# EBonura/bonnie-32

Measured on AMD Instinct MI355X. Metric: Mtriangles/s + Mpixels/s, 1M-tri synthetic scene @ 2560x1920, higher is better.
Workload: dtype f32+i32 (exact-order f32 setup/barycentrics, integer snap and RGB555 colour tail); 1 GPU; C3: 1000000 tris @ 2560x1920, 256x256 8-bit atlas, affine+snap+RGB555 dither, painter's; triangles_drawn=485525, fragments=9622635, parallelism=single GPU

## Files before the change

### bonnie-32_amd/csrc/b32_api.hip

```cpp
#include "b32_host.h"

extern "C" {

const char* b32_strerror(int code) {
    switch (code) {
        case B32_OK: return "ok";
        case B32_E_ARG: return "invalid argument";
        case B32_E_INDEX: return "face references a vertex index out of range";
        case B32_E_NAN_KEY: return "NaN painter's-sort key";
        case B32_E_HIP: return "HIP runtime error";
        case B32_E_UNSUPPORTED: return "setting outside the supported hot-path scope";
        case B32_E_NO_DEVICE: return "no HIP device (the rasterizer has no CPU fallback)";
        case B32_E_FRAME_DROPPED: return "an earlier frame in flight ran out of buffer space and drew nothing (deep asynchronous mode)";
        case B32_E_BAND_TIMEOUT: return "a band exchange wait gave up: another rank did not publish / release its frame in time (the frame may hold stale rows)";
        default: return "unknown error";
    }
}

int b32_create(int device, b32_ctx** out) {
    if (!out) return B32_E_ARG;
    *out = nullptr;
    int n = 0;
    if (hipGetDeviceCount(&n) != hipSuccess || n <= 0 || device < 0 || device >= n) return B32_E_NO_DEVICE;
    b32_ctx* c = new b32_ctx();
// ... 32 lines not shown
    if (c->side) (void)hipStreamDestroy(c->side);
    if (c->ev_created) for (auto& fr : c->ev) for (auto& e : fr) if (e) (void)hipEventDestroy(e);
    c->lines.release(); c->prims.release(); c->world.release(); c->gizmo.release();
    if (c->world_counts) (void)hipFree(c->world_counts);
    if (c->gizmo_counts) (void)hipFree(c->gizmo_counts);
    for (hipEvent_t e : c->world_ev) if (e) (void)hipEventDestroy(e);
    c->pick_tab.release();
    if (c->pick_words) (void)hipFree(c->pick_words);
    if (c->pick_host) (void)hipHostFree(c->pick_host);
    for (hipEvent_t e : c->pick_tev) if (e) (void)hipEventDestroy(e);
    if (c->hover_bits) (void)hipFree(c->hover_bits);
    if (c->hover_words) (void)hipFree(c->hover_words);
    for (hipEvent_t e : c->hover_tev) if (e) (void)hipEventDestroy(e);
    if (c->own_stream) (void)hipStreamDestroy(c->own_stream);
    if (c->stage_host) (void)hipHostFree(c->stage_host);
    for (hipEvent_t e : c->dl_ev) if (e) (void)hipEventDestroy(e);
    if (c->dl_stream) { (void)hipStreamSynchronize(c->dl_stream); (void)hipStreamDestroy(c->dl_stream); }
    for (hipEvent_t e : c->dl_snap) if (e) (void)hipEventDestroy(e);
    for (uint32_t* q : c->dl_stage) if (q) (void)hipFree(q);
    for (uint32_t k = 0; k < b32_ctx::PICK_RING; ++k) {
        if (c->pick_res[k]) (void)hipFree(c->pick_res[k]);
        for (hipEvent_t e : { c->pick_done[k], c->pick_left[k] }) if (e) (void)hipEventDestroy(e);
    }
    delete c;
}

int b32_last_hip_error(const b32_ctx* c) { return c ? c->last_hip : 0; }
#ifndef B32_SRC_DIGEST
#define B32_SRC_DIGEST "unknown-digest!!"
#endif
// ... 651 lines not shown
    if (c->hover_timed && k < cap && hipEventSynchronize(c->hover_tev[1]) == hipSuccess &&
        hipEventElapsedTime(&hover_ms, c->hover_tev[0], c->hover_tev[1]) == hipSuccess) {
        names[k] = "hover"; ms[k] = hover_ms; ++k;
    }
    return (int)k;
}

}

extern "C" int b32_set_fragment_counting(b32_ctx* c, int on) {
    if (!c) return B32_E_ARG;
    c->count_fragments = on ? 1 : 0;
    return B32_OK;
}
extern "C" unsigned long long b32_route_count(const b32_ctx* c, int which) {
    if (c && which == 7) return c->pipelined_frames;
    if (c && which == 8) return c->lds_atlas_frames;
    if (c && which == 9) return c->wire_tile_frames;
    if (c && which == 10) return c->span_cover_frames;
    if (c && which == 11) return c->flag_join_frames;
    if (c && which == 12) return c->event_join_frames;
    if (c && which == 13) return c->poll_join_frames;
    if (c && which == 14) return c->lines.tile_batches;
    if (c && which == 15) return c->lines.scan_batches;
    if (c && which == 16) return c->prims.tile_batches;
    if (c && which == 17) return c->prims.scan_batches;
    if (c && which == 18) return c->world_tile_batches;
    if (c && which == 19) return c->world_scan_batches;
    return (c && which >= 0 && which < 8) ? c->routes[which] : 0ull;
}
// ... 84 lines not shown
```

### bonnie-32_amd/csrc/b32_device.h

```cpp
#pragma once
#include <hip/hip_runtime.h>
#include <stdint.h>
#include "../../include/b32raster.h"

namespace b32 {

constexpr int TILE_W = 64;
constexpr int TILE_H = 64;
constexpr int TILE_STRIDE = 72;
constexpr int FILL_THREADS = 1024;
constexpr int FILL_WAVES = FILL_THREADS / 64;
constexpr uint32_t KEY_INVALID = 0xFFFFFFFFu;

namespace K {
constexpr int      FRAC_BITS = 12;
constexpr float    ONE_F = (float)(1 << FRAC_BITS);
constexpr uint32_t UNR_ENTRIES = 257, UNR_INDEX_OFFSET = 256, UNR_NUMERATOR = 262144, UNR_ROUND_ADD = 1, UNR_ROUND_DIV = 2;
constexpr int32_t  UNR_SUBTRACT = 257;
constexpr uint32_t DIV_D16_SHIFT = 16, DIV_INDEX_SHIFT = 7, DIV_INDEX_MAX = 256, DIV_NR1_SHIFT = 8, DIV_NR2_SHIFT = 8, DIV_SHIFT_BASE = 36;
constexpr uint64_t DIV_INDEX_BIAS = 0x7FC0, DIV_U_ADD = 0x101, DIV_NR1_CONST = 0x2000080, DIV_NR2_CONST = 0x80;
constexpr float    PF_DISTANCE = 5.0f, PF_SCALE = 4.0f, PF_VIEWPORT_DIV = 2.0f, PF_VIEWPORT_FRAC = 0.75f;
constexpr int32_t  PF_DENOM_GUARD = 256;
constexpr float    P_DISTANCE = 5.0f, P_US_SUB = 1.0f, P_VIEWPORT_DIV = 2.0f, P_VIEWPORT_FRAC = 0.75f, P_DENOM_GUARD = 0.001f;
constexpr float    NEAR_PLANE = 0.1f;
// ... 102 lines not shown
    uint32_t pairs_overflow;
    uint32_t tile_cursor;
    uint32_t list_demand;
    uint32_t need_global_sort;
    uint32_t wire_overflow;
    uint32_t sticky;
    unsigned long long fragments;
};

struct Stamps { unsigned long long t[8]; };
struct Events { uint32_t bad_index, nan_opaque, nan_transparent, overflow, long_transparent, setup_done ,
                join_abort ,
                fill_started ,
                wbin_done ,
                poll_done ,
                poll_lost , _pad[5]; };
__device__ __forceinline__ Events* events_of(Ctrl* ctrl) { return reinterpret_cast<Events*>(reinterpret_cast<unsigned char*>(ctrl) + 128); }
enum { ST_SETUP = 0, ST_BIN = 1, ST_FILL = 2, ST_WIRE = 3, ST_END = 4,
       ST_CLK0 = 5, ST_CLK1 = 6, ST_CLKW = 7 };
__device__ __forceinline__ void phase_stamp(Ctrl* ctrl, int k) {
    if (blockIdx.x == 0 && threadIdx.x == 0) {
        unsigned long long* t = reinterpret_cast<Stamps*>(ctrl + 1)->t;
        if (!t[k]) t[k] = wall_clock64();
    }
}

constexpr uint32_t LOCAL_SORT_CAP = 2048;

struct CamFx {
    int32_t px, py, pz, bx[3], by[3], bz[3];
    int32_t vs, half_w, half_h;
// ... 292 lines not shown
    const uint32_t* spans;
    const uint32_t* partials;
    const uint32_t* texmask;
    uint32_t mask_lds_words;
    uint32_t clear_on, clear_rgba;
    uint32_t clear_depth;
    uint32_t narrow_only;
    const uint8_t* atlas0;
    uint32_t atlas_idx_bytes;
    uint32_t stagger;
    uint32_t span_cover;
    uint32_t join_seq, join_patience;
    uint32_t start_seq;
    uint32_t start_defer;
    uint32_t prio64;
#ifdef B32_TIMELINE
    unsigned long long* dbg;
#endif
};
void launch_fill(hipStream_t s, const FillArgs& a, int n_cu, hipEvent_t after_cover = nullptr);
size_t fill_lds_tex_budget();
constexpr uint32_t ATLAS_CLUT_BYTES = 512;
uint32_t fill_lds_atlas_room(bool wide);

}
```

### bonnie-32_amd/csrc/b32_fill.hip

```cpp
#include "b32_cover.h"
#include "b32_shade_tile.h"

namespace b32 {

constexpr uint32_t RQ_WORDS = 64, RQ_BYTES = RQ_WORDS * 4;
static_assert(2 * (4 * LDS_TILE_BYTES + LDS_MISC_BYTES + 8 * RQ_BYTES + 511) / 512 * 512 <= 160 * 1024, "two 8-wave workgroups per CU");

template <int NT>
__device__ __forceinline__ void reduce_setup_counters(const FillArgs& a, uint32_t* misc, uint32_t tid, uint32_t lane) {
    if (tid < 5) misc[8 + tid] = 0;
    __syncthreads();
    const uint32_t npart = (a.fp.nf + 255) / 256;
    uint32_t acc[5] = { 0, 0, 0, 0, 0 };
    for (uint32_t b = tid; b < npart; b += NT)
#pragma unroll
        for (int k = 0; k < 5; ++k) acc[k] += a.partials[b * 8 + k];
#pragma unroll
    for (int k = 0; k < 5; ++k) {
        const uint32_t tot = (uint32_t)__builtin_amdgcn_readlane((int)dpp_add_scan(acc[k]), 63);
        if (lane == 0 && tot) atomicAdd(&misc[8 + k], tot);
    }
    __syncthreads();
    if (tid == 0) {
        const uint32_t t[5] = { misc[8], misc[9], misc[10], misc[11], misc[12] };
// ... 35 lines not shown
    if (tid == 0) {
        Events* ev = events_of(a.ctrl);
        const unsigned long long t0 = wall_clock64();
        uint32_t lost = 0, waited = 0;
        while (__hip_atomic_fetch_add(&ev->poll_done, 0u, __ATOMIC_RELAXED, __HIP_MEMORY_SCOPE_AGENT) != a.join_seq) {
            if (wall_clock64() - t0 > (unsigned long long)a.join_patience) { lost = 1; break; }
            waited = 1;
            __builtin_amdgcn_s_sleep(32);
        }
        if (lost) { atomicOr(&a.ctrl->sticky, 8u); (void)__hip_atomic_exchange(&ev->poll_lost, a.join_seq, __ATOMIC_RELAXED, __HIP_MEMORY_SCOPE_AGENT); }
        if (waited) __builtin_amdgcn_fence(__ATOMIC_ACQUIRE, "agent");
        misc[7] = lost;
    }
    __syncthreads();
    return misc[7] != 0;
}

template <int NT>
__device__ __forceinline__ TexDesc stage_texture(const FillArgs& a, unsigned char* dst_bytes, uint32_t tid) {
    const TexDesc lds_desc = a.tex[0];
    const uint4* src = reinterpret_cast<const uint4*>(a.texels + lds_desc.offset);
    uint4* dst = reinterpret_cast<uint4*>(dst_bytes);
    const uint32_t nq = (a.lds_tex_texels + 7) / 8;
    for (uint32_t i = tid; i < nq; i += NT) dst[i] = src[i];
    return lds_desc;
}

template <int NT>
__device__ __forceinline__ void leave_undrawn(const FillArgs& a, uint32_t ntiles, uint32_t tid, uint32_t redraw, bool publish) {
    if (a.direct_bin) {
// ... 187 lines not shown
    const bool join_lost = (P64 && a.join_seq) ? join_setup(a, misc, tid) : false;
    phase_stamp(a.ctrl, ST_FILL);
    uint32_t pre_span = 0xFFFFFFFFu, pre_key = 0u;
    if (P64 && a.inline_bin && tid < fp.nf && !join_lost) { pre_span = a.spans[tid]; if (a.gather_blend) pre_key = a.keys[tid]; }
    if (P64 && EXACT && a.mask_lds_words) {
        uint32_t* ml = tilebuf + 2 * TILE_H * TILE_STRIDE;
        for (uint32_t i = tid; i < a.mask_lds_words; i += NT) ml[i] = a.texmask[i];
        ltex = reinterpret_cast<const uint16_t*>(ml);
    }
    bool reduce_late = false;
    if (P64 && (a.inline_bin || a.direct_bin)) {
        bool reduce = a.inline_bin != 0, join_abort = join_lost;
        uint32_t redraw = 0;
        if (a.direct_bin) {
            const Events* ev = events_of(a.ctrl);
            reduce = ev->bad_index == a.epoch || ev->nan_opaque == a.epoch || ev->nan_transparent == a.epoch;
            redraw = (ev->overflow == a.epoch ? 2u : 0u) | (ev->long_transparent == a.epoch ? 1u : 0u);
            join_abort = join_lost || ev->join_abort == a.epoch;
            reduce_late = !reduce && blockIdx.x == 0;
        }
        if (tid == 0) misc[6] = 0;
        __syncthreads();
        if (reduce && !join_abort) reduce_setup_counters<NT>(a, misc, tid, lane);
        if (join_abort) {
            leave_undrawn<NT>(a, ntiles, tid, 0u, false);
            return;
        }
        if (misc[6] || redraw) {
            leave_undrawn<NT>(a, ntiles, tid, redraw, !misc[6]);
            return;
        }
    } else {
        if (a.ctrl->abort || (P64 && a.ctrl->need_global_sort)) {
// ... 66 lines not shown
    }
#ifdef B32_TIMELINE
    if (P64 && a.dbg && lane < 32 && B32_DBG_SLOTS(tilebuf)[lane]) atomicAdd(a.dbg + 1 + 4 * 8192 + lane, B32_DBG_SLOTS(tilebuf)[lane]);
#endif
    if (P64 && blockIdx.x == 0 && tid == 0) {
        unsigned long long* st = reinterpret_cast<Stamps*>(a.ctrl + 1)->t;
        st[ST_CLK0] = clk_entry; st[ST_CLK1] = (unsigned long long)clock64(); st[ST_CLKW] = wall_clock64();
    }
    if (P64 && reduce_late) { __syncthreads(); reduce_setup_counters<NT>(a, misc, tid, lane); }
    if (EXACT && !ZMODE) publish_fragments<NW>(a, smem, frag_count, tid, lane, wave);
}

template <int TEXMODE, bool EXACT, int NT, bool ZMODE, bool FMT8 = false, bool P64 = false, int PLAIN = 0>
__global__ __launch_bounds__(NT) __attribute__((amdgpu_waves_per_eu((P64 && NT == 512 && !PLAIN) ? B32_P64_WAVES : 4))) void k_cover(FillArgs a_in) {
    cover_body<TEXMODE, EXACT, NT, ZMODE, FMT8, P64, PLAIN>(a_in);
}

#ifndef B32_PLAIN_CAP
#define B32_PLAIN_CAP 56
#endif
__global__ __launch_bounds__(512) __attribute__((amdgpu_waves_per_eu(4), amdgpu_num_vgpr(B32_PLAIN_CAP))) void k_cover_plain(FillArgs a_in) {
    cover_body<0, false, 512, false, false, true, 1>(a_in);
}
__global__ __launch_bounds__(512) __attribute__((amdgpu_waves_per_eu(4), amdgpu_num_vgpr(56))) void k_cover_plain_z(FillArgs a_in) {
    cover_body<0, false, 512, true, false, true, 1>(a_in);
}
__global__ __launch_bounds__(512) __attribute__((amdgpu_waves_per_eu(4), amdgpu_num_vgpr(56))) void k_cover_plain8(FillArgs a_in) {
    cover_body<0, false, 512, false, true, true, 2>(a_in);
}
#ifndef B32_LIT_VGPR
#define B32_LIT_VGPR 56
#endif
__global__ __launch_bounds__(512) __attribute__((amdgpu_waves_per_eu(4), amdgpu_num_vgpr(B32_LIT_VGPR))) void k_cover_lit(FillArgs a_in) {
    cover_body<0, false, 512, true, false, true, 3>(a_in);
}

#ifdef B32_TIMELINE
static unsigned long long* g_timeline = nullptr;
extern "C" int b32_debug_timeline(unsigned long long* out, unsigned cap_words) {
    if (!g_timeline) return 0;
    (void)hipDeviceSynchronize();
    (void)hipMemcpy(out, g_timeline, (size_t)cap_words * 8, hipMemcpyDeviceToHost);
    return 1;
}
#endif
template <bool EXACT, bool ZMODE, bool FMT8>
static void launch_p64(hipStream_t s, const FillArgs& a_in, uint32_t ntiles, int n_cu, bool wide) {
    FillArgs a = a_in;
    const size_t atlas = a.atlas_idx_bytes ? (((size_t)ATLAS_CLUT_BYTES + a.atlas_idx_bytes + 15) & ~(size_t)15) : 0;
// ... 115 lines not shown
```

### bonnie-32_amd/csrc/b32_frame.hip

```cpp
#include "b32_host.h"

static void swap_with(b32_ctx* c, FrameSet& a) { std::swap(c->cur, a); }
static void rotate_sets(b32_ctx* c) {
    swap_with(c, c->alt[0]);
    if (c->n_sets == 3) std::swap(c->alt[0], c->alt[1]);
}
static void unrotate_sets(b32_ctx* c) {
    if (c->n_sets == 3) std::swap(c->alt[0], c->alt[1]);
    swap_with(c, c->alt[0]);
}
static int pipeline_ensure(b32_ctx* c) {
    if (!c->side) {
        int prio_least = 0, prio_greatest = 0;
        (void)hipDeviceGetStreamPriorityRange(&prio_least, &prio_greatest);
        HIPCHK(c, hipStreamCreateWithPriority(&c->side, hipStreamNonBlocking, prio_least));
        HIPCHK(c, hipEventCreateWithFlags(&c->ev_main, hipEventDisableTiming));
        HIPCHK(c, hipEventCreateWithFlags(&c->ev_wbin, hipEventDisableTiming));
        HIPCHK(c, hipEventCreateWithFlags(&c->cur.ev_setup, hipEventDisableTiming));
        for (FrameSet& a : c->alt) HIPCHK(c, hipEventCreateWithFlags(&a.ev_setup, hipEventDisableTiming));
        c->side_dirty = true;
    }
    for (uint32_t k = 0; k + 1 < c->n_sets; ++k) {
        FrameSet& a = c->alt[k];
        if (!a.d_ctrl) {
            HIPCHK(c, hipMalloc(reinterpret_cast<void**>(&a.d_ctrl), sizeof(Ctrl) + sizeof(Stamps) + sizeof(Events)));
            HIPCHK(c, hipMemsetAsync(a.d_ctrl, 0, sizeof(Ctrl) + sizeof(Stamps) + sizeof(Events), c->stream));
            c->side_dirty = true;
        }
        if (a.cap_work < c->cap_work || !a.crecs) {
            HIPCHK(c, hipStreamSynchronize(c->stream));
            a.release();
            const size_t n = c->cap_work;
            int rc;
            if ((rc = ensure_plain(c, a.keys0, n))) return rc;
// ... 334 lines not shown
    const bool join_small = !c->frame_batched && (c->join_stream != s || c->join_ok);
    c->pipe_hint = r.direct_bin && (ntiles > 2u * (uint32_t)c->n_cu || c->frame_batched || join_small);
    if (!c->pipe_hint) c->pipelined = false;
    c->last_local_sort = r.local_sort || r.want_prio64;
    c->last_exact = r.ordered_all ? true : (r.exact_cov && !fp.zmode);
    c->last_direct = r.direct_bin;
    if (c->scene.nf == 0) {
        HIPCHK(c, hipMemsetAsync(c->cur.d_ctrl, 0, offsetof(Ctrl, sticky), s));
        HIPCHK(c, hipMemsetAsync(&c->cur.d_ctrl->fragments, 0, sizeof(unsigned long long), s));
        HIPCHK(c, hipMemsetAsync(c->cur.d_ctrl + 1, 0, sizeof(Stamps), s));
    }
    const float *pos12 = nullptr, *attr12 = nullptr;
    if ((rc = frame_positions(c, fp, pos12, attr12))) return fail(rc);

    hipStream_t ss = s;
    if (c->pipelined) {
        if (c->side_dirty) { HIPCHK(c, hipEventRecord(c->ev_main, s)); HIPCHK(c, hipStreamWaitEvent(c->side, c->ev_main, 0)); c->side_dirty = false; }
        ss = c->side;
        c->pipelined_frames++;
        uint32_t polled_tiles = 0, polled_groups = 0, polled_seq = 0;
        for (const auto& co : c->cover_of) if (co.ctrl && co.ctrl == c->alt[0].d_ctrl) { polled_tiles = co.tiles; polled_groups = co.groups; polled_seq = co.seq; }
        const bool start_gate = polled_tiles && polled_seq && c->alt[0].d_ctrl;
        if (!start_gate) { HIPCHK(c, hipEventRecord(c->ev_main, s)); HIPCHK(c, hipStreamWaitEvent(c->side, c->ev_main, 0)); }
        uint32_t gate_need = 0;
        if (c->gate_permille && polled_tiles && c->alt[0].d_ctrl) {
            const uint32_t groups = polled_groups, tiles = polled_tiles;
            const uint32_t pre = tiles > groups ? tiles - groups : 0u;
            const uint32_t need = c->gate_permille > 1000u ? (uint32_t)((uint64_t)(c->gate_permille - 1000u) * pre / 1000u)
                                                           : pre + (uint32_t)((uint64_t)(c->gate_permille - 1u) * groups / 1000u);
            gate_need = need;
        }
        const uint32_t start_patience = c->start_lost ? 200000u : 200000000u;
        c->start_lost = false;
        if (gate_need || start_gate) launch_gate(ss, c->alt[0].d_ctrl, gate_need, 30000u , start_gate ? polled_seq : 0u, c->cur.d_ctrl, start_patience);
    }
    const bool wire_on = fp.wire_collect && c->scene.nf;
    bool wire_binned = false, wire_polled = false;
    WireArgs wa{};
    if (wire_on) {
        wa.tris = c->cur.wire; wa.nf = c->scene.nf; wa.table_owner = c->wire_owner; wa.table_first = c->wire_first;
        wa.table_mask = c->cap_wire_table ? (uint32_t)(c->cap_wire_table - 1) : 0;
        wa.fb = c->fb; wa.zbuf = (c->zbuf && c->zbuf_valid) ? c->zbuf : nullptr;
        wa.width = c->width; wa.height = c->height; wa.band_y0 = c->band_y0; wa.band_y1 = c->band_y1; wa.ctrl = c->cur.d_ctrl;
        if (++c->wire_seq == 0) c->wire_seq = 1;
        wa.epoch = c->wire_seq;
        if (!(c->route_off & B32_ROUTE_WIRE_TILES) && c->cur.wire_fill && c->band_y1 > c->band_y0) {
            wa.tile_yb = (c->band_y0 / WIRE_TH) * WIRE_TH; wa.tiles_x = (c->width + TILE_W - 1) / TILE_W;
            wa.tiles_y = (c->band_y1 - wa.tile_yb + WIRE_TH - 1) / WIRE_TH;
// ... 4 lines not shown
    launch_setup(ss, fp, c->scene.d_verts, c->scene.d_faces, c->scene.d_tex, c->d_lights, lset, c->frame_table, c->frame_places, RecArrays{ c->cur.crecs, c->cur.srecs, c->cur.xrecs }, r.db, c->cur.shades, c->cur.keys0,
                 r.direct_bin ? nullptr : c->cur.spans , c->cur.partials, c->cur.d_ctrl, c->cur.wire, c->n_cu, pos12, attr12, c->cur.face_of);
    uint32_t poll_seq = 0, poll_patience = 0;
    const bool poll_batched = c->pipelined && c->frame_batched && c->join_ok && (r.direct_bin || r.want_inline) && !wire_front && !r.ordered_all &&
                              ntiles && 8u * ntiles <= 5u * (uint32_t)c->n_cu && !(c->route_off & B32_ROUTE_WIDE_GROUPS);
    if (poll_batched) {
        const bool lose_flag = (c->inject & 1u) != 0;
        c->inject &= ~1u;
        if (++c->join_seq == 0) c->join_seq = 1;
        launch_flag_poll(c->side, c->cur.d_ctrl, lose_flag ? c->join_seq ^ 0x40000000u : c->join_seq);
        poll_seq = c->join_seq; poll_patience = lose_flag ? 200000u : 200000000u;
        c->flag_join_frames++; c->poll_join_frames++;
    } else if (c->pipelined && r.direct_bin && c->join_ok && !c->frame_batched) {
        const bool lose_flag = (c->inject & 1u) != 0;
        c->inject &= ~1u;
        launch_flag(c->side, c->cur.d_ctrl, lose_flag ? c->epoch ^ 0x40000000u : c->epoch);
        launch_join(s, c->cur.d_ctrl, c->epoch, lose_flag ? 200000u : 200000000u );
        c->flag_join_frames++;
    } else if (c->pipelined) {
        hipError_t e1 = hipEventRecord(c->cur.ev_setup, c->side);
        if (e1 == hipSuccess) e1 = hipStreamWaitEvent(s, c->cur.ev_setup, 0);
        if (e1 != hipSuccess) { (void)hipStreamSynchronize(c->side); c->last_hip = (int)e1; return B32_E_HIP; }
        c->event_join_frames++;
    }
    if (c->pipelined && wire_on && wa.tile_fill) {
        launch_wire_bin(c->side, wa, wire_back, wire_front, true);
        if (wire_back) { launch_flag_wbin(c->side, c->cur.d_ctrl, wa.epoch); wire_polled = true; }
        else HIPCHK(c, hipEventRecord(c->ev_wbin, c->side));
        wire_binned = true;
    }
    c->cur.in_flight = true;
    if (prof_all) HIPCHK(c, hipEventRecord(ev[1], s));
// ... 11 lines not shown
        if (prof_all) HIPCHK(c, hipEventRecord(ev[2], s));
        r.prio64 = r.inline_bin = true;
    } else if (r.want_prio64) {
        if (prof_all) HIPCHK(c, hipEventRecord(ev[2], s));
        r.prio64 = launch_bin_spans(s, fp, c->cur.spans, r.with_class ? c->cur.keys0 : nullptr, c->cur.partials, c->cur.d_ctrl, sc, (uint32_t)c->cap_pairs, c->ranges,
                                    c->tile_mid, BLEND_SORT_CAP, c->pvals[0]);
    }
    if (!r.prio64 && (rc = bin_keyed(c, fp, r, sc, prof_all ? ev[2] : nullptr, cur))) return rc;
    c->routes[r.direct_bin ? 0 : r.inline_bin ? 1 : r.prio64 ? 2 : 3]++;
    const bool direct_safe = r.direct_bin && r.db.cap_opaque >= c->scene.nf && (!r.with_class || c->scene.blend_faces <= BLEND_SORT_CAP);
    c->pending_may_redraw = !(r.inline_bin || direct_safe);
    if (prof_fill) HIPCHK(c, hipEventRecord(ev[3], s));

    FillArgs fa = fill_args(c, fp, r, cur, wire_front);
    if (++c->fill_seq == 0) c->fill_seq = 1;
    fa.start_seq = c->fill_seq;
    fa.join_seq = poll_seq; fa.join_patience = poll_patience;
    const uint32_t start_seq_meant = fa.start_seq;
    if ((c->inject & 2u) && fa.prio64 && !wire_front && !r.ordered_all && ntiles) { c->inject &= ~2u; fa.start_seq = 0; c->start_lost = true; }
    fa.start_defer = (fa.prio64 && !wire_front && !r.ordered_all && ntiles > 2u * (uint32_t)c->n_cu && fa.gather_blend) ? 1u : 0u;
    if (c->clear_pending) {
        const bool has_z = c->zbuf && c->zbuf_valid;
        if (r.prio64 && !wire_front && !r.ordered_all && (!has_z || fp.zmode) && c->scene.nf && ntiles && c->clear_y0 == c->band_y0 && c->clear_y1 == c->band_y1) {
            fa.clear_on = 1; fa.clear_rgba = c->clear_rgba; fa.clear_depth = (has_z && fp.zmode) ? 1u : 0u; c->clear_pending = false;
        } else if ((rc = flush_clear(c))) return rc;
    }
    if (fa.atlas_idx_bytes && !wire_front && !r.ordered_all) c->lds_atlas_frames++;
    if (fa.span_cover && !wire_front && !r.ordered_all) c->span_cover_frames++;
    launch_fill(s, fa, c->n_cu, prof_fill ? ev[4] : nullptr);

    if (wire_on) {
        if (wire_binned && !wire_polled) HIPCHK(c, hipStreamWaitEvent(s, c->ev_wbin, 0));
        launch_wire(s, wa, wire_back, wire_front, wire_binned, wire_polled ? c->cur.d_ctrl : nullptr, wa.epoch);
    }
    if (prof_fill) { if (prof_all) HIPCHK(c, hipEventRecord(ev[5], s)); c->ev_frames++; }
    c->last_cover_tiles = (r.prio64 && !wire_front && !r.ordered_all) ? ntiles : 0u;
    c->last_cover_groups = std::min<uint32_t>(ntiles, (uint32_t)c->n_cu * 2u);
    {
        b32_ctx::CoverOf* slot = &c->cover_of[0];
        for (auto& co : c->cover_of) { if (co.ctrl == c->cur.d_ctrl) { slot = &co; break; } if (!co.ctrl) slot = &co; }
        *slot = { c->cur.d_ctrl, c->last_cover_tiles, c->last_cover_groups, c->last_cover_tiles ? start_seq_meant : 0u };
    }
    HIPCHK(c, hipGetLastError());
// ... 54 lines not shown
int b32_frame_finish(b32_ctx* c, B32Timings* out) {
    if (!c) return B32_E_ARG;
    (void)hipSetDevice(c->device);
    if (out) memset(out, 0, sizeof(*out));
    const bool later_clear = c->frame_pending && c->clear_pending;
    const uint32_t lc_rgba = c->clear_rgba, lc_y0 = c->clear_y0, lc_y1 = c->clear_y1;
    if (later_clear) c->clear_pending = false;
    struct ClearAfter {
        b32_ctx* c; bool on; uint32_t rgba, y0, y1;
        ~ClearAfter() { if (on) { c->clear_pending = true; c->clear_rgba = rgba; c->clear_y0 = y0; c->clear_y1 = y1; (void)flush_clear(c); (void)hipStreamSynchronize(c->stream); } }
    } clear_after{ c, later_clear, lc_rgba, lc_y0, lc_y1 };
    const bool no_redraw = c->frame_pending && c->pending_superseded && !later_clear;
    if (!later_clear) { const int rcf = flush_clear(c); if (rcf) return rcf; }
    if (!c->frame_pending) {
        HIPCHK(c, hipStreamSynchronize(c->stream));
        const int d = c->deferred_rc; c->deferred_rc = 0;
        return d;
    }
    for (int attempt = 0; attempt < 5; ++attempt) {
        if (stage_ensure(c)) {
            launch_ctrl_out(c->stream, c->cur.d_ctrl, static_cast<unsigned char*>(c->stage_dev) + STAGE_CTRL_OFF);
            HIPCHK(c, hipStreamSynchronize(c->stream));
            std::memcpy(&c->h_ctrl, c->stage_host + STAGE_CTRL_OFF, sizeof(Ctrl));
            std::memcpy(&c->h_stamps, c->stage_host + STAGE_CTRL_OFF + sizeof(Ctrl), sizeof(Stamps));
        } else {
            unsigned char tmp[sizeof(Ctrl) + sizeof(Stamps)];
            HIPCHK(c, hipMemcpyAsync(tmp, c->cur.d_ctrl, sizeof(tmp), hipMemcpyDeviceToHost, c->stream));
            HIPCHK(c, hipStreamSynchronize(c->stream));
            std::memcpy(&c->h_ctrl, tmp, sizeof(Ctrl)); std::memcpy(&c->h_stamps, tmp + sizeof(Ctrl), sizeof(Stamps));
            c->h_stamps.t[ST_END] = 0;
// ... 24 lines not shown
        const size_t n = (size_t)c->h_ctrl.pairs_overflow + c->h_ctrl.pairs_overflow / 4 + 1024;
        int rc;
        for (int i = 0; i < 2; ++i) { if ((rc = ensure_plain(c, c->pkeys[i], n))) return rc; if ((rc = ensure_plain(c, c->pvals[i], n))) return rc; }
        c->cap_pairs = n;
        if (no_redraw) break;
        c->routes[6]++;
        c->ev_frames = 0;
        c->redrawing = true;
        rc = enqueue_frame(c, &c->last_cam, &c->last_settings, c->last_has_fog ? &c->last_fog : nullptr);
        c->redrawing = false;
        if (rc) return rc;
    }
    c->frame_pending = false;
    c->pending_superseded = false;
    c->cur.in_flight = false;
    collect_events(c);
    uint32_t sticky = c->h_ctrl.sticky;
    if (sticky) HIPCHK(c, hipMemsetAsync(&c->cur.d_ctrl->sticky, 0, sizeof(uint32_t), c->stream));
    if (sticky) c->side_dirty = true;
    for (FrameSet& o : c->alt) if (o.in_flight && o.d_ctrl) {
        Ctrl other;
        HIPCHK(c, hipMemcpy(&other, o.d_ctrl, sizeof(Ctrl), hipMemcpyDeviceToHost));
        o.in_flight = false;
        uint32_t st2 = other.sticky;
        if (other.pairs_overflow || other.need_global_sort) st2 += 0x100u;
        if (other.sticky) HIPCHK(c, hipMemsetAsync(&o.d_ctrl->sticky, 0, sizeof(uint32_t), c->stream));
        if (other.pairs_overflow || other.need_global_sort) {
            HIPCHK(c, hipMemsetAsync(&o.d_ctrl->pairs_overflow, 0, sizeof(uint32_t), c->stream));
            HIPCHK(c, hipMemsetAsync(&o.d_ctrl->need_global_sort, 0, sizeof(uint32_t), c->stream));
        }
// ... 43 lines not shown
```

### bonnie-32_amd/csrc/b32_host.h

```cpp
#pragma once
#include "b32_device.h"
#include <algorithm>
#include <cstdio>
#include <chrono>
#include <cstring>
#include <vector>

using namespace b32;
#ifndef B32_MIN_TILE_H
#define B32_MIN_TILE_H 8
#endif

namespace {
constexpr int EV_RING = 64;
constexpr int EV_PER_FRAME = 6;
}

struct FrameSet {
    uint32_t* keys0 = nullptr; CovRec* crecs = nullptr; ShadeRec* srecs = nullptr; AuxRec* xrecs = nullptr;
    uint32_t* spans = nullptr; uint32_t* partials = nullptr; size_t cap_work = 0;
    uint32_t* face_of = nullptr;
    float* shades = nullptr; size_t cap_shades = 0;
    uint32_t* direct_lists = nullptr; size_t cap_direct = 0;
    uint32_t* tile_fill = nullptr; size_t cap_tile_fill = 0;
    WireTri* wire = nullptr; size_t cap_wire = 0;
    uint32_t *wire_fill = nullptr, *wire_lists = nullptr; size_t cap_wire_tiles = 0;
    unsigned long long wire_grid = 0;
    Ctrl* d_ctrl = nullptr;
    hipEvent_t ev_setup = nullptr;
    bool in_flight = false;
    void release() {
        for (void* p : { (void*)keys0, (void*)crecs, (void*)srecs, (void*)xrecs, (void*)spans, (void*)face_of, (void*)partials, (void*)shades,
                         (void*)direct_lists, (void*)tile_fill, (void*)wire, (void*)wire_fill, (void*)wire_lists }) if (p) (void)hipFree(p);
        FrameSet e; e.d_ctrl = d_ctrl; e.ev_setup = ev_setup; e.in_flight = in_flight;
        *this = e;
    }
};

constexpr uint32_t LINE_RING = 4;
template <class Rec>
struct DrawPassState {
    Rec* host[LINE_RING] = {}; size_t cap_host[LINE_RING] = {}; hipEvent_t ev[LINE_RING] = {}; uint32_t slot = 0;
    Rec* dev = nullptr; size_t cap_dev = 0;
    uint32_t *counters = nullptr, *lists = nullptr, *long_list = nullptr; size_t cap_tiles = 0; uint32_t parity = 0;
    unsigned long long tile_batches = 0, scan_batches = 0;
    void release() {
        for (uint32_t k = 0; k < LINE_RING; ++k) { if (ev[k]) (void)hipEventDestroy(ev[k]); if (host[k]) (void)hipHostFree(host[k]); }
        for (void* p : { (void*)dev, (void*)counters, (void*)lists, (void*)long_list }) if (p) (void)hipFree(p);
    }
// ... 45 lines not shown
    uint32_t n_sets_user = 0;
    uint32_t n_sets = 2;
    bool side_dirty = true;
    hipStream_t join_stream = nullptr; bool join_ok = false;
    uint32_t gate_permille = 0;
    uint32_t wire_seq = 0;
    bool start_lost = false;
    uint32_t join_seq = 0;
    uint32_t fill_seq = 0;
    bool pipe_hint = true;
    struct CoverOf { const Ctrl* ctrl; uint32_t tiles, groups, seq; } cover_of[3] = {};
    uint32_t last_cover_tiles = 0, last_cover_groups = 0;
    bool pipelined = false;
    unsigned long long pipelined_frames = 0;
    unsigned long long flag_join_frames = 0, event_join_frames = 0, poll_join_frames = 0;
    uint32_t inject = 0;

    uint32_t width = 0, height = 0;
    uint32_t* fb_own = nullptr; size_t fb_own_px = 0;
    uint32_t* fb = nullptr; bool fb_external = false;
    uint32_t band_y0 = 0, band_y1 = 0; bool band_set = false;
    float* zbuf = nullptr; size_t cap_zbuf = 0; bool zbuf_valid = false;

    void* band_fb_ipc = nullptr; uint32_t* band_sync_own = nullptr; uint32_t* band_sync = nullptr;
    uint32_t band_rank = 0; bool band_attached = false;

    b32_scene scene;
    int count_fragments = 0;
    bool last_exact = false;

// ... 167 lines not shown
```

### bonnie-32_amd/rasterizer.py

```python
import ctypes as C

import numpy as np

from . import abi
from . import rtypes as T


class B32Error(RuntimeError):
    def __init__(self, code, where=""):
        self.code = code
        msg = abi.load_library().b32_strerror(code).decode()
        super().__init__(f"{where}: {msg} (code {code})" if where else f"{msg} (code {code})")


def _chk(rc, where=""):
    if rc != abi.B32_OK:
        raise B32Error(rc, where)


def place_vertices(vertices, cos_f, sin_f, world_pos):
    v = np.array(vertices, dtype=abi.VERTEX_DTYPE, copy=True)
    c, s = np.float32(cos_f), np.float32(sin_f)
    w = np.asarray(world_pos, np.float32).reshape(3)
    with np.errstate(all="ignore"):
# ... 453 lines not shown
    def synchronize(self):
        _chk(self.lib.b32_synchronize(self.h), "b32_synchronize")

    def set_profiling(self, level):
        _chk(self.lib.b32_set_profiling(self.h, level), "b32_set_profiling")

    def set_profiling_stride(self, every):
        _chk(self.lib.b32_set_profiling_stride(self.h, int(every)), "b32_set_profiling_stride")

    def set_async_depth(self, deep):
        _chk(self.lib.b32_set_async_depth(self.h, int(deep)), "b32_set_async_depth")

    ROUTES = ("direct_bin", "inline_bin", "counting_sort", "keyed", "redraw_region", "redraw_global_sort", "redraw_pairs", "pipelined", "lds_atlas", "wire_tiles", "span_cover",
              "flag_join", "event_join", "poll_join", "line_tiles", "line_scan", "prim_tiles", "prim_scan")
    WORLD_ROUTES = ("world_tiles", "world_scan")

    ROUTE_SORT_FREE, ROUTE_CUT_TILES, ROUTE_INLINE_BIN, ROUTE_DIRECT_BIN, ROUTE_WIDE_GROUPS, ROUTE_PACKED_STREAMS, ROUTE_PIPELINE, ROUTE_TEX_CACHE, ROUTE_BATCH, ROUTE_LDS_ATLAS, ROUTE_WIRE_TILES, ROUTE_SPAN_COVER, ROUTE_STAGGER, ROUTE_LINE_TILES, ROUTE_PRIM_TILES = 1, 2, 4, 8, 16, 32, 64, 128, 256, 512, 1024, 2048, 4096, 8192, 16384

    def frame_begin(self, camera, settings):
        cam = camera.pack()
        st, keep = settings.pack()
        self._frame_keep = (cam, st, keep)
        _chk(self.lib.b32_frame_begin(self.h, C.byref(cam), C.byref(st)), "b32_frame_begin")

    def frame_add(self, scene, ambient=None, backface_cull=None, backface_wireframe=None, fog=None, placement=None):
        st = self._frame_keep[1]
        p = abi.B32MeshParams()
        p.ambient = float(st.ambient if ambient is None else ambient)
        p.backface_cull = int(st.backface_cull if backface_cull is None else bool(backface_cull))
        p.backface_wireframe = int(st.backface_wireframe if backface_wireframe is None else bool(backface_wireframe))
        fg = T.pack_fog(fog)
        p.has_fog = 0 if fg is None else 1
# ... 224 lines not shown
        cam = camera.pack()
        o = _pack_ortho(ortho)
        n = C.c_uint32()
        _chk(self.lib.b32_gizmo_project_batch(self.h, C.byref(cam), C.byref(o) if o is not None else None, arr.ctypes.data if len(arr) else None,
                                              len(arr), int(width), int(height), out.ctypes.data if cap else None, cap, C.byref(n)),
             "gizmo_project_batch")
        return out[:int(n.value)]

    def set_routes(self, off_mask):
        _chk(self.lib.b32_set_routes(self.h, int(off_mask)), "b32_set_routes")

    def set_cheap_threshold(self, den):
        _chk(self.lib.b32_set_cheap_threshold(self.h, int(den)), "b32_set_cheap_threshold")

    def route_counts(self):
        return {n: int(self.lib.b32_route_count(self.h, i)) for i, n in enumerate(self.ROUTES + self.WORLD_ROUTES)}

    def debug_inject(self, what):
        _chk(self.lib.b32_debug_inject(self.h, int(what)), "b32_debug_inject")

    def set_fragment_counting(self, on):
        _chk(self.lib.b32_set_fragment_counting(self.h, int(on)), "b32_set_fragment_counting")

    def last_kernel_times(self):
        names = (C.c_char_p * 8)()
        ms = (C.c_float * 8)()
        n = self.lib.b32_last_kernel_times(self.h, names, ms, 8)
        return {names[i].decode(): float(ms[i]) for i in range(n)}

    BAND_SHARE_BYTES = 96

# ... 641 lines not shown
```

### include/b32raster.h

```cpp
#ifndef B32RASTER_H
#define B32RASTER_H

#include <stddef.h>
#include <stdint.h>

#ifdef __cplusplus
extern "C" {
#endif

#define B32_OK             0
#define B32_E_ARG         -1
#define B32_E_INDEX       -2
#define B32_E_NAN_KEY     -3
#define B32_E_HIP         -4
#define B32_E_UNSUPPORTED -5
#define B32_E_NO_DEVICE   -6
#define B32_E_FRAME_DROPPED -7
#define B32_E_BAND_TIMEOUT -8

#define B32_BLEND_OPAQUE      0
#define B32_BLEND_AVERAGE     1
#define B32_BLEND_ADD         2
#define B32_BLEND_SUBTRACT    3
#define B32_BLEND_ADD_QUARTER 4
// ... 148 lines not shown
unsigned long long b32_route_count(const b32_ctx* ctx, int which);
#define B32_ROUTE_SORT_FREE   1u
#define B32_ROUTE_CUT_TILES   2u
#define B32_ROUTE_INLINE_BIN  4u
#define B32_ROUTE_DIRECT_BIN  8u
#define B32_ROUTE_WIDE_GROUPS 16u
#define B32_ROUTE_PACKED_STREAMS 32u
#define B32_ROUTE_TEX_CACHE   128u
#define B32_ROUTE_BATCH       256u
#define B32_ROUTE_LDS_ATLAS   512u
#define B32_ROUTE_WIRE_TILES  1024u
#define B32_ROUTE_SPAN_COVER  2048u
#define B32_ROUTE_STAGGER     4096u
#define B32_ROUTE_LINE_TILES  8192u
#define B32_ROUTE_PRIM_TILES 16384u
#define B32_ROUTE_PIPELINE    64u
int b32_set_routes(b32_ctx* ctx, uint32_t off_mask);
int b32_set_cheap_threshold(b32_ctx* ctx, uint32_t den);

typedef struct b32_scene b32_scene;
int b32_scene_create(b32_ctx* ctx, b32_scene** out);
void b32_scene_destroy(b32_ctx* ctx, b32_scene* slot);
int b32_scene_swap(b32_ctx* ctx, b32_scene* slot);

typedef struct B32MeshParams {
    float   ambient;
    uint8_t backface_cull, backface_wireframe, has_fog, _pad;
    B32Fog  fog;
} B32MeshParams;
int b32_frame_begin(b32_ctx* ctx, const B32Camera* camera, const B32Settings* base_settings);
// ... 202 lines not shown
```

Before: 9932 Mtriangles/s.

## Let predecessor fill kernel hand over setup-done join to next frame

In pipelined direct-bin frames, the last workgroup of the previous fill kernel now waits for the next frame's setup flag and marks it joined. This replaces the separate join kernel launch on the main stream. A host-mapped coherent ring of slots carries the epoch and patience to the device, and the fill kernel falls back to polling when no predecessor handed over. The aim is to drop one kernel launch and one stream bubble between frames, at the cost of more cross-kernel signalling and timeout paths.

Result: no change. 9902 Mtriangles/s (-0.3%).

```diff
diff --git a/bonnie-32_amd/csrc/b32_api.hip b/bonnie-32_amd/csrc/b32_api.hip
--- a/bonnie-32_amd/csrc/b32_api.hip
+++ b/bonnie-32_amd/csrc/b32_api.hip
@@ -70,6 +70,7 @@
     for (hipEvent_t e : c->hover_tev) if (e) (void)hipEventDestroy(e);
     if (c->own_stream) (void)hipStreamDestroy(c->own_stream);
     if (c->stage_host) (void)hipHostFree(c->stage_host);
+    if (c->pred_ring) (void)hipHostFree(c->pred_ring);
     for (hipEvent_t e : c->dl_ev) if (e) (void)hipEventDestroy(e);
     if (c->dl_stream) { (void)hipStreamSynchronize(c->dl_stream); (void)hipStreamDestroy(c->dl_stream); }
     for (hipEvent_t e : c->dl_snap) if (e) (void)hipEventDestroy(e);
@@ -751,6 +752,16 @@
     return B32_OK;
 }
 extern "C" unsigned long long b32_route_count(const b32_ctx* c, int which) {
+    if (c && (which == 20 || which == 21)) {
+        (void)hipSetDevice(c->device);
+        if (hipStreamSynchronize(c->stream) != hipSuccess) return 0ull;
+        unsigned long long n = 0;
+        for (const FrameSet* a : { &c->cur, &c->alt[0], &c->alt[1] }) {
+            Events ev;
+            if (a->d_ctrl && hipMemcpy(&ev, reinterpret_cast<const unsigned char*>(a->d_ctrl) + sizeof(Ctrl) + sizeof(Stamps), sizeof(Events), hipMemcpyDeviceToHost) == hipSuccess) n += which == 20 ? ev.n_pred : ev.n_poll;
+        }
+        return n;
+    }
     if (c && which == 7) return c->pipelined_frames;
     if (c && which == 8) return c->lds_atlas_frames;
     if (c && which == 9) return c->wire_tile_frames;
diff --git a/bonnie-32_amd/csrc/b32_device.h b/bonnie-32_amd/csrc/b32_device.h
--- a/bonnie-32_amd/csrc/b32_device.h
+++ b/bonnie-32_amd/csrc/b32_device.h
@@ -140,7 +140,21 @@
                 fill_started ,
                 wbin_done ,
                 poll_done ,
-                poll_lost , _pad[5]; };
+                poll_lost ,
+                pred_left ,
+                pred_joined ,
+                n_pred, n_poll ,
+                _pad0;
+                unsigned long long pred_seen ;
+                uint32_t _pad[6]; };
+static_assert(sizeof(Events) == 96, "Events layout (one allocation with Ctrl and Stamps)");
+struct PredSlot {
+    unsigned long long key;
+    unsigned long long payload;
+    unsigned long long closed;
+    unsigned long long _pad;
+};
+constexpr uint32_t PRED_RING = 1024;
 __device__ __forceinline__ Events* events_of(Ctrl* ctrl) { return reinterpret_cast<Events*>(reinterpret_cast<unsigned char*>(ctrl) + 128); }
 enum { ST_SETUP = 0, ST_BIN = 1, ST_FILL = 2, ST_WIRE = 3, ST_END = 4,
        ST_CLK0 = 5, ST_CLK1 = 6, ST_CLKW = 7 };
@@ -463,6 +477,11 @@
     uint32_t start_seq;
     uint32_t start_defer;
     uint32_t prio64;
+    Ctrl* pred_next;
+    PredSlot* pred_slot;
+    uint32_t pred_seq;
+    uint32_t pred_base;
+    uint32_t pred_join;
 #ifdef B32_TIMELINE
     unsigned long long* dbg;
 #endif
diff --git a/bonnie-32_amd/csrc/b32_fill.hip b/bonnie-32_amd/csrc/b32_fill.hip
--- a/bonnie-32_amd/csrc/b32_fill.hip
+++ b/bonnie-32_amd/csrc/b32_fill.hip
@@ -73,6 +73,67 @@
     }
     __syncthreads();
     return misc[7] != 0;
+}
+
+__device__ __forceinline__ bool join_pred(const FillArgs& a, uint32_t* misc, uint32_t tid) {
+    Events* ev = events_of(a.ctrl);
+    const bool by_pred = ev->pred_joined == a.epoch;
+    if (by_pred || ev->join_abort == a.epoch) {
+        if (by_pred && blockIdx.x == 0 && tid == 0) atomicAdd(&ev->n_pred, 1u);
+        return false;
+    }
+    if (tid == 0) {
+        const unsigned long long t0 = wall_clock64();
+        uint32_t lost = 0;
+        while ((int32_t)(__hip_atomic_fetch_add(&ev->setup_done, 0u, __ATOMIC_RELAXED, __HIP_MEMORY_SCOPE_AGENT) - a.epoch) < 0) {
+            if (wall_clock64() - t0 > (unsigned long long)a.join_patience) { lost = 1; break; }
+            __builtin_amdgcn_s_sleep(32);
+        }
+        if (lost) { atomicOr(&a.ctrl->sticky, 8u); (void)__hip_atomic_exchange(&ev->join_abort, a.epoch, __ATOMIC_RELAXED, __HIP_MEMORY_SCOPE_AGENT); }
+        else __builtin_amdgcn_fence(__ATOMIC_ACQUIRE, "agent");
+        if (blockIdx.x == 0) atomicAdd(&ev->n_poll, 1u);
+        misc[7] = lost;
+    }
+    __syncthreads();
+    return misc[7] != 0;
+}
+
+__device__ __forceinline__ void close_handover(const FillArgs& a) {
+    if (!a.pred_next || threadIdx.x != 0) return;
+    Events* mine = events_of(a.ctrl);
+    const uint32_t left = __hip_atomic_fetch_add(&mine->pred_left, 1u, __ATOMIC_RELAXED, __HIP_MEMORY_SCOPE_AGENT) + 1u - a.pred_base;
+    if (left == 1u && gridDim.x > 1u) {
+        const unsigned long long key = __hip_atomic_load(&a.pred_slot->key, __ATOMIC_RELAXED, __HIP_MEMORY_SCOPE_SYSTEM);
+        if ((uint32_t)(key >> 32) == a.pred_seq && (uint32_t)key) __hip_atomic_store(&mine->pred_seen, key, __ATOMIC_RELAXED, __HIP_MEMORY_SCOPE_AGENT);
+        return;
+    }
+    if (left != gridDim.x) return;
+    Events* next = events_of(a.pred_next);
+    const unsigned long long seen = __hip_atomic_fetch_add(&mine->pred_seen, 0ull, __ATOMIC_RELAXED, __HIP_MEMORY_SCOPE_AGENT);
+    uint32_t flag = __hip_atomic_fetch_add(&next->setup_done, 0u, __ATOMIC_RELAXED, __HIP_MEMORY_SCOPE_AGENT);
+    uint32_t epoch = (uint32_t)seen;
+    if ((uint32_t)(seen >> 32) != a.pred_seq) {
+        const unsigned long long key = __hip_atomic_load(&a.pred_slot->key, __ATOMIC_RELAXED, __HIP_MEMORY_SCOPE_SYSTEM);
+        epoch = (uint32_t)key;
+        if ((uint32_t)(key >> 32) != a.pred_seq || !epoch) {
+            __hip_atomic_store(&a.pred_slot->closed, (unsigned long long)a.pred_seq, __ATOMIC_RELAXED, __HIP_MEMORY_SCOPE_SYSTEM);
+            return;
+        }
+    }
+    if ((int32_t)(flag - epoch) < 0) {
+        const unsigned long long pay = __hip_atomic_load(&a.pred_slot->payload, __ATOMIC_RELAXED, __HIP_MEMORY_SCOPE_SYSTEM);
+        const unsigned long long patience = (uint32_t)pay == epoch ? pay >> 32 : 200000000ull, t0 = wall_clock64();
+        do {
+            if (wall_clock64() - t0 > patience) {
+                atomicOr(&a.pred_next->sticky, 8u);
+                (void)__hip_atomic_exchange(&next->join_abort, epoch, __ATOMIC_RELAXED, __HIP_MEMORY_SCOPE_AGENT);
+                return;
+            }
+            __builtin_amdgcn_s_sleep(4);
+            flag = __hip_atomic_fetch_add(&next->setup_done, 0u, __ATOMIC_RELAXED, __HIP_MEMORY_SCOPE_AGENT);
+        } while ((int32_t)(flag - epoch) < 0);
+    }
+    __hip_atomic_store(&next->pred_joined, epoch, __ATOMIC_RELAXED, __HIP_MEMORY_SCOPE_AGENT);
 }
 
 template <int NT>
@@ -290,9 +351,10 @@
         uint32_t redraw = 0;
         if (a.direct_bin) {
             const Events* ev = events_of(a.ctrl);
+            const bool pred_lost = a.pred_join ? join_pred(a, misc, tid) : false;
             reduce = ev->bad_index == a.epoch || ev->nan_opaque == a.epoch || ev->nan_transparent == a.epoch;
             redraw = (ev->overflow == a.epoch ? 2u : 0u) | (ev->long_transparent == a.epoch ? 1u : 0u);
-            join_abort = join_lost || ev->join_abort == a.epoch;
+            join_abort = join_lost || pred_lost || ev->join_abort == a.epoch;
             reduce_late = !reduce && blockIdx.x == 0;
         }
         if (tid == 0) misc[6] = 0;
@@ -389,6 +451,7 @@
 template <int TEXMODE, bool EXACT, int NT, bool ZMODE, bool FMT8 = false, bool P64 = false, int PLAIN = 0>
 __global__ __launch_bounds__(NT) __attribute__((amdgpu_waves_per_eu((P64 && NT == 512 && !PLAIN) ? B32_P64_WAVES : 4))) void k_cover(FillArgs a_in) {
     cover_body<TEXMODE, EXACT, NT, ZMODE, FMT8, P64, PLAIN>(a_in);
+    if (P64) close_handover(a_in);
 }
 
 #ifndef B32_PLAIN_CAP
@@ -396,18 +459,22 @@
 #endif
 __global__ __launch_bounds__(512) __attribute__((amdgpu_waves_per_eu(4), amdgpu_num_vgpr(B32_PLAIN_CAP))) void k_cover_plain(FillArgs a_in) {
     cover_body<0, false, 512, false, false, true, 1>(a_in);
+    close_handover(a_in);
 }
 __global__ __launch_bounds__(512) __attribute__((amdgpu_waves_per_eu(4), amdgpu_num_vgpr(56))) void k_cover_plain_z(FillArgs a_in) {
     cover_body<0, false, 512, true, false, true, 1>(a_in);
+    close_handover(a_in);
 }
 __global__ __launch_bounds__(512) __attribute__((amdgpu_waves_per_eu(4), amdgpu_num_vgpr(56))) void k_cover_plain8(FillArgs a_in) {
     cover_body<0, false, 512, false, true, true, 2>(a_in);
+    close_handover(a_in);
 }
 #ifndef B32_LIT_VGPR
 #define B32_LIT_VGPR 56
 #endif
 __global__ __launch_bounds__(512) __attribute__((amdgpu_waves_per_eu(4), amdgpu_num_vgpr(B32_LIT_VGPR))) void k_cover_lit(FillArgs a_in) {
     cover_body<0, false, 512, true, false, true, 3>(a_in);
+    close_handover(a_in);
 }
 
 #ifdef B32_TIMELINE
diff --git a/bonnie-32_amd/csrc/b32_frame.hip b/bonnie-32_amd/csrc/b32_frame.hip
--- a/bonnie-32_amd/csrc/b32_frame.hip
+++ b/bonnie-32_amd/csrc/b32_frame.hip
@@ -18,6 +18,14 @@
         HIPCHK(c, hipEventCreateWithFlags(&c->ev_wbin, hipEventDisableTiming));
         HIPCHK(c, hipEventCreateWithFlags(&c->cur.ev_setup, hipEventDisableTiming));
         for (FrameSet& a : c->alt) HIPCHK(c, hipEventCreateWithFlags(&a.ev_setup, hipEventDisableTiming));
+        void* ring = nullptr;
+        if (hipHostMalloc(&ring, PRED_RING * sizeof(PredSlot), hipHostMallocMapped | hipHostMallocCoherent) == hipSuccess) {
+            void* ring_dev = nullptr;
+            std::memset(ring, 0, PRED_RING * sizeof(PredSlot));
+            if (hipHostGetDevicePointer(&ring_dev, ring, 0) == hipSuccess) { c->pred_ring = static_cast<PredSlot*>(ring); c->pred_ring_dev = static_cast<PredSlot*>(ring_dev); }
+            else (void)hipHostFree(ring);
+        }
+        (void)hipGetLastError();
         c->side_dirty = true;
     }
     for (uint32_t k = 0; k + 1 < c->n_sets; ++k) {
@@ -382,14 +390,19 @@
     if ((rc = frame_positions(c, fp, pos12, attr12))) return fail(rc);
 
     hipStream_t ss = s;
+    const bool pred_shape = r.direct_bin && !c->frame_batched && !fp.wire_collect && !wire_front && !r.ordered_all && !r.with_class && ntiles && c->scene.nf &&
+                            !(c->route_off & B32_ROUTE_PRED_JOIN);
+    bool pred_join = false;
+    uint32_t pred_patience = 0;
     if (c->pipelined) {
+        bool side_waits_main = c->side_dirty;
         if (c->side_dirty) { HIPCHK(c, hipEventRecord(c->ev_main, s)); HIPCHK(c, hipStreamWaitEvent(c->side, c->ev_main, 0)); c->side_dirty = false; }
         ss = c->side;
         c->pipelined_frames++;
         uint32_t polled_tiles = 0, polled_groups = 0, polled_seq = 0;
         for (const auto& co : c->cover_of) if (co.ctrl && co.ctrl == c->alt[0].d_ctrl) { polled_tiles = co.tiles; polled_groups = co.groups; polled_seq = co.seq; }
         const bool start_gate = polled_tiles && polled_seq && c->alt[0].d_ctrl;
-        if (!start_gate) { HIPCHK(c, hipEventRecord(c->ev_main, s)); HIPCHK(c, hipStreamWaitEvent(c->side, c->ev_main, 0)); }
+        if (!start_gate) { HIPCHK(c, hipEventRecord(c->ev_main, s)); HIPCHK(c, hipStreamWaitEvent(c->side, c->ev_main, 0)); side_waits_main = true; }
         uint32_t gate_need = 0;
         if (c->gate_permille && polled_tiles && c->alt[0].d_ctrl) {
             const uint32_t groups = polled_groups, tiles = polled_tiles;
@@ -400,6 +413,15 @@
         }
         const uint32_t start_patience = c->start_lost ? 200000u : 200000000u;
         c->start_lost = false;
+        if (pred_shape && c->join_ok && !side_waits_main && c->pred_frames < PRED_RING && c->pred.armed && c->pred.stream == s && c->pred.next == c->cur.d_ctrl && c->pred_ring) {
+            PredSlot& sl = c->pred_ring[c->pred.seq % PRED_RING];
+            if (__atomic_load_n(&sl.closed, __ATOMIC_RELAXED) != c->pred.seq) {
+                pred_patience = (c->inject & 1u) ? 200000u : 200000000u;
+                __atomic_store_n(&sl.payload, ((unsigned long long)pred_patience << 32) | c->epoch, __ATOMIC_RELAXED);
+                __atomic_store_n(&sl.key, ((unsigned long long)c->pred.seq << 32) | c->epoch, __ATOMIC_RELEASE);
+                pred_join = true;
+            }
+        }
         if (gate_need || start_gate) launch_gate(ss, c->alt[0].d_ctrl, gate_need, 30000u , start_gate ? polled_seq : 0u, c->cur.d_ctrl, start_patience);
     }
     const bool wire_on = fp.wire_collect && c->scene.nf;
@@ -434,8 +456,8 @@
     } else if (c->pipelined && r.direct_bin && c->join_ok && !c->frame_batched) {
         const bool lose_flag = (c->inject & 1u) != 0;
         c->inject &= ~1u;
-        launch_flag(c->side, c->cur.d_ctrl, lose_flag ? c->epoch ^ 0x40000000u : c->epoch);
-        launch_join(s, c->cur.d_ctrl, c->epoch, lose_flag ? 200000u : 200000000u );
+        launch_flag(c->side, c->cur.d_ctrl, lose_flag ? (pred_join ? c->epoch - 0x40000000u : c->epoch ^ 0x40000000u) : c->epoch);
+        if (!pred_join) launch_join(s, c->cur.d_ctrl, c->epoch, lose_flag ? 200000u : 200000000u );
         c->flag_join_frames++;
     } else if (c->pipelined) {
         hipError_t e1 = hipEventRecord(c->cur.ev_setup, c->side);
@@ -477,8 +499,10 @@
 
     FillArgs fa = fill_args(c, fp, r, cur, wire_front);
     if (++c->fill_seq == 0) c->fill_seq = 1;
+    if (c->pred_frames < PRED_RING) c->pred_frames++;
     fa.start_seq = c->fill_seq;
     fa.join_seq = poll_seq; fa.join_patience = poll_patience;
+    if (pred_join) { fa.pred_join = 1; fa.join_patience = pred_patience; }
     const uint32_t start_seq_meant = fa.start_seq;
     if ((c->inject & 2u) && fa.prio64 && !wire_front && !r.ordered_all && ntiles) { c->inject &= ~2u; fa.start_seq = 0; c->start_lost = true; }
     fa.start_defer = (fa.prio64 && !wire_front && !r.ordered_all && ntiles > 2u * (uint32_t)c->n_cu && fa.gather_blend) ? 1u : 0u;
@@ -490,6 +514,13 @@
     }
     if (fa.atlas_idx_bytes && !wire_front && !r.ordered_all) c->lds_atlas_frames++;
     if (fa.span_cover && !wire_front && !r.ordered_all) c->span_cover_frames++;
+    c->pred.armed = false;
+    if (pred_shape && c->pred_ring_dev && c->alt[0].d_ctrl) {
+        fa.pred_next = c->alt[0].d_ctrl; fa.pred_seq = start_seq_meant; fa.pred_slot = c->pred_ring_dev + start_seq_meant % PRED_RING;
+        fa.pred_base = c->cur.pred_left;
+        c->cur.pred_left += std::min<uint32_t>(ntiles, (uint32_t)c->n_cu * 2u);
+        c->pred = { true, start_seq_meant, fa.pred_next, s };
+    }
     launch_fill(s, fa, c->n_cu, prof_fill ? ev[4] : nullptr);
 
     if (wire_on) {
@@ -574,6 +605,7 @@
     if (!later_clear) { const int rcf = flush_clear(c); if (rcf) return rcf; }
     if (!c->frame_pending) {
         HIPCHK(c, hipStreamSynchronize(c->stream));
+        c->pred_frames = 0;
         const int d = c->deferred_rc; c->deferred_rc = 0;
         return d;
     }
@@ -628,6 +660,7 @@
     c->frame_pending = false;
     c->pending_superseded = false;
     c->cur.in_flight = false;
+    c->pred_frames = 0;
     collect_events(c);
     uint32_t sticky = c->h_ctrl.sticky;
     if (sticky) HIPCHK(c, hipMemsetAsync(&c->cur.d_ctrl->sticky, 0, sizeof(uint32_t), c->stream));
diff --git a/bonnie-32_amd/csrc/b32_host.h b/bonnie-32_amd/csrc/b32_host.h
--- a/bonnie-32_amd/csrc/b32_host.h
+++ b/bonnie-32_amd/csrc/b32_host.h
@@ -29,10 +29,11 @@
     Ctrl* d_ctrl = nullptr;
     hipEvent_t ev_setup = nullptr;
     bool in_flight = false;
+    uint32_t pred_left = 0;
     void release() {
         for (void* p : { (void*)keys0, (void*)crecs, (void*)srecs, (void*)xrecs, (void*)spans, (void*)face_of, (void*)partials, (void*)shades,
                          (void*)direct_lists, (void*)tile_fill, (void*)wire, (void*)wire_fill, (void*)wire_lists }) if (p) (void)hipFree(p);
-        FrameSet e; e.d_ctrl = d_ctrl; e.ev_setup = ev_setup; e.in_flight = in_flight;
+        FrameSet e; e.d_ctrl = d_ctrl; e.ev_setup = ev_setup; e.in_flight = in_flight; e.pred_left = pred_left;
         *this = e;
     }
 };
@@ -108,6 +109,9 @@
     bool pipelined = false;
     unsigned long long pipelined_frames = 0;
     unsigned long long flag_join_frames = 0, event_join_frames = 0, poll_join_frames = 0;
+    PredSlot* pred_ring = nullptr; PredSlot* pred_ring_dev = nullptr;
+    uint32_t pred_frames = 0;
+    struct PredOf { bool armed = false; uint32_t seq = 0; Ctrl* next = nullptr; hipStream_t stream = nullptr; } pred;
     uint32_t inject = 0;
 
     uint32_t width = 0, height = 0;
diff --git a/bonnie-32_amd/rasterizer.py b/bonnie-32_amd/rasterizer.py
--- a/bonnie-32_amd/rasterizer.py
+++ b/bonnie-32_amd/rasterizer.py
@@ -491,8 +491,9 @@
     ROUTES = ("direct_bin", "inline_bin", "counting_sort", "keyed", "redraw_region", "redraw_global_sort", "redraw_pairs", "pipelined", "lds_atlas", "wire_tiles", "span_cover",
               "flag_join", "event_join", "poll_join", "line_tiles", "line_scan", "prim_tiles", "prim_scan")
     WORLD_ROUTES = ("world_tiles", "world_scan")
-
-    ROUTE_SORT_FREE, ROUTE_CUT_TILES, ROUTE_INLINE_BIN, ROUTE_DIRECT_BIN, ROUTE_WIDE_GROUPS, ROUTE_PACKED_STREAMS, ROUTE_PIPELINE, ROUTE_TEX_CACHE, ROUTE_BATCH, ROUTE_LDS_ATLAS, ROUTE_WIRE_TILES, ROUTE_SPAN_COVER, ROUTE_STAGGER, ROUTE_LINE_TILES, ROUTE_PRIM_TILES = 1, 2, 4, 8, 16, 32, 64, 128, 256, 512, 1024, 2048, 4096, 8192, 16384
+    PRED_ROUTES = ("joined_by_predecessor", "joined_by_poll")
+
+    ROUTE_SORT_FREE, ROUTE_CUT_TILES, ROUTE_INLINE_BIN, ROUTE_DIRECT_BIN, ROUTE_WIDE_GROUPS, ROUTE_PACKED_STREAMS, ROUTE_PIPELINE, ROUTE_TEX_CACHE, ROUTE_BATCH, ROUTE_LDS_ATLAS, ROUTE_WIRE_TILES, ROUTE_SPAN_COVER, ROUTE_STAGGER, ROUTE_LINE_TILES, ROUTE_PRIM_TILES, ROUTE_PRED_JOIN = 1, 2, 4, 8, 16, 32, 64, 128, 256, 512, 1024, 2048, 4096, 8192, 16384, 32768
 
     def frame_begin(self, camera, settings):
         cam = camera.pack()
@@ -747,7 +748,7 @@
         _chk(self.lib.b32_set_cheap_threshold(self.h, int(den)), "b32_set_cheap_threshold")
 
     def route_counts(self):
-        return {n: int(self.lib.b32_route_count(self.h, i)) for i, n in enumerate(self.ROUTES + self.WORLD_ROUTES)}
+        return {n: int(self.lib.b32_route_count(self.h, i)) for i, n in enumerate(self.ROUTES + self.WORLD_ROUTES + self.PRED_ROUTES)}
 
     def debug_inject(self, what):
         _chk(self.lib.b32_debug_inject(self.h, int(what)), "b32_debug_inject")
diff --git a/include/b32raster.h b/include/b32raster.h
--- a/include/b32raster.h
+++ b/include/b32raster.h
@@ -186,6 +186,7 @@
 #define B32_ROUTE_STAGGER     4096u
 #define B32_ROUTE_LINE_TILES  8192u
 #define B32_ROUTE_PRIM_TILES 16384u
+#define B32_ROUTE_PRED_JOIN  32768u
 #define B32_ROUTE_PIPELINE    64u
 int b32_set_routes(b32_ctx* ctx, uint32_t off_mask);
 int b32_set_cheap_threshold(b32_ctx* ctx, uint32_t den);
```
